# 87003697/DynamiCrafter

Measured on AMD Instinct MI355X. Metric: frames/sec (and denoising-step ms), 16f@576x1024, DDIM 50, higher is better.
Workload: dtype bf16; 1 GPU; inference_1024_v1.0.yaml: 1 clip/GPU, 16 frames, latent 72x128, DDIM 50 uniform_trailing eta=1, CFG 7.5 batched (cond+uncond), guidance_rescale 0.7, v-param+ZTSNR+dynamic rescale, hipGraph-captured step; clips_per_gpu=1, parallelism=dp1 over 1 distinct clips (no data-path collective), conditioning=local (1 rank), outputs_finite=True

## Files before the change

### dynamicrafter_amd/csrc/ff_fused.hip

```cpp
#include "attn_parts.h"
#include "dc_common.h"
#include "dcrafter_hip.h"
#include "lds_stage.h"
#include <stdint.h>
#include <type_traits>

namespace {

constexpr int FD = 320;
constexpr int FM = 4 * FD;
constexpr int FCH = 32;
constexpr int FNCH = FM / FCH;
constexpr int FBM = 128;
constexpr int W1_STAGE = 64 * FD * 2;
constexpr int W2_STAGE = FD * FCH * 2;
constexpr int W2_RING = 3;
constexpr int FF_LDS = 2 * W1_STAGE + W2_RING * W2_STAGE + 4 * 2048 + 2 * FM * 4;
static_assert(FF_LDS <= 160 * 1024, "LDS");

#ifdef DC_FF_STAMPS
__device__ unsigned long long g_ff_stamps[8];
#define FF_STAMP(i) do { asm volatile("s_waitcnt lgkmcnt(0)" ::: "memory"); const unsigned long long t__ = __builtin_readcyclecounter(); \
                         st_acc[i] += t__ - st_last; st_last = t__; } while (0)
#else
#define FF_STAMP(i) do { } while (0)
#endif

#ifdef DC_FF_GELU_ERF
#define FF_GELU(x) gelu_erf_f(x)
#else
#define FF_GELU(x) gelu_phi_f(x)
#endif

constexpr int LCH = 32;
constexpr int LW_STAGE = LCH * FD * 2;

template <int ROW_BYTES, int TILE_BYTES, bool PIN = true>
__device__ __forceinline__ void xs_piece_offsets(unsigned (&vo)[5], int wave, int lane) {
#pragma unroll
    for (int i = 0; i < 5; ++i) {
        const int u = wave * 5 + i;
        const int t = u >> 2, g = u & 3;
        vo[i] = (unsigned)((g * 8 + (lane >> 3)) * ROW_BYTES + t * TILE_BYTES + (((lane & 7) ^ ((g * 4 + (lane >> 4)) & 7)) << 4));
        if constexpr (PIN) asm volatile("" : "+v"(vo[i]));
    }
}
__device__ __forceinline__ unsigned xs_stage_dst(unsigned lds_base, int stage_off, int wave, int i) {
    return lds_base + stage_off + (wave * 5 + i) * 1024;
}
__device__ __forceinline__ void xs_issue_stage(unsigned lds_base, int stage_off, int wave, const unsigned (&vo)[5], uint64_t sbase) {
#pragma unroll
    for (int i = 0; i < 5; ++i) lds_dma16_sbase(xs_stage_dst(lds_base, stage_off, wave, i), vo[i], sbase);
}

template <int ROWS = 32>
__device__ __forceinline__ bf16x8_t xs_read_frag(const char* stage, int kk, int row, int fh) {
    return *(lds_vfrag_t*)((lds_char_t*)stage + (kk >> 2) * (ROWS * 128) + lds_off128(row, (kk & 3) * 2 + fh));
}

template <int PD, int NK, class Issue>
__device__ __forceinline__ void xs_stage_mma(const char* stage, const bf16x8_t (&xf)[NK], int k0, f32x16_t& acc, int fr, int fh,
                                             Issue&& issue) {
    bf16x8_t wr[PD];
#pragma unroll
    for (int kk = 0; kk < PD; ++kk) wr[kk] = xs_read_frag(stage, kk, fr, fh);
#pragma unroll
    for (int kk = 0; kk < FD / 16; ++kk) {
        bf16x8_t f = wr[kk % PD];
        if (kk + PD < FD / 16) wr[kk % PD] = xs_read_frag(stage, kk + PD, fr, fh);
        asm volatile("" : "+v"(f));
        acc = __builtin_amdgcn_mfma_f32_32x32x16_bf16(f, xf[k0 + kk], acc, 0, 0, 0);
        if (kk < 5) issue(kk);
    }
}

struct XsRowsLinear {
    int m0, M;
    __device__ __forceinline__ bool ok(int r) const { return m0 + r < M; }
    __device__ __forceinline__ size_t operator()(int r) const { return (size_t)(m0 + r); }
    __device__ __forceinline__ size_t clamped(int r) const { int m = m0 + r; if (m >= M) m = M - 1; return (size_t)m; }
};
struct XsRowsGather {
    int b, HW, p0;
    __device__ __forceinline__ bool ok(int) const { return true; }
    __device__ __forceinline__ size_t operator()(int r) const { return ((size_t)(b * 16 + (r & 15))) * HW + p0 + (r >> 4); }
    __device__ __forceinline__ size_t clamped(int r) const { return (*this)(r); }
};

template <int NK>
__device__ __forceinline__ void xs_load_rows(bf16x8_t (&xf)[NK], const bf16_t* xrow) {
#pragma unroll
    for (int kk = 0; kk < NK; ++kk) xf[kk] = *reinterpret_cast<const bf16x8_t*>(xrow + kk * 16);
}

__device__ __forceinline__ void xs_stage_ln_affine(float* lns, int KD, const float* g, const float* b, int tid) {
    for (int i = tid; i < KD; i += 256) { lns[i] = g[i]; lns[KD + i] = b[i]; }
}
__device__ __forceinline__ void xs_stage_gn_affine(float* lns, int KD, const float* g, const float* b, const float2* stats, int groups,
                                                   int tid) {
    for (int i = tid; i < KD; i += 256) {
        const float2 st = stats[i / (KD / groups)];
        const float a = g[i] * st.y;
        lns[i] = a; lns[KD + i] = b[i] - st.x * a;
    }
}
__device__ __forceinline__ void xs_stage_bias(float* bls, const float* bias, int N, int tid) {
    for (int i = tid; i < N; i += 256) bls[i] = bias[i];
}

__device__ __forceinline__ uint2* xs_patch_acc(char* ebuf, int fr, int fh, int q) {
    return reinterpret_cast<uint2*>(ebuf + fr * 64 + (((2 * q + fh) ^ (((fr >> 1) & 3) << 1)) << 3));
}
__device__ __forceinline__ u32x4_t* xs_patch_row(char* ebuf, int r, int rc) {
    return reinterpret_cast<u32x4_t*>(ebuf + r * 64 + ((rc ^ ((r >> 1) & 3)) << 4));
}
template <class Rows>
__device__ __forceinline__ void xs_load_chunk_rows(u32x4_t (&d)[2], const bf16_t* R, int ldr, const Rows& rows, int n0, int lane) {
#pragma unroll
    for (int t = 0; t < 2; ++t)
        d[t] = *reinterpret_cast<const u32x4_t*>(R + rows.clamped(t * 16 + (lane >> 2)) * ldr + n0 + (lane & 3) * 8);
}
__device__ __forceinline__ void xs_add_bf16x8(u32x4_t& d, const u32x4_t& rr) {
#pragma unroll
    for (int e = 0; e < 4; ++e) d[e] = add_bf2(d[e], rr[e]);
}
__device__ __forceinline__ void xs_add_bf16x4(float4& bv, uint2 rv) {
    bv.x += __uint_as_float(rv.x << 16); bv.y += __uint_as_float(rv.x & 0xffff0000u);
    bv.z += __uint_as_float(rv.y << 16); bv.w += __uint_as_float(rv.y & 0xffff0000u);
}
__device__ __forceinline__ uint2 xs_pack_acc(const f32x16_t& acc, int q, const float4& bv) {
    uint2 pk;
    pk.x = pack_bf2(acc[4 * q] + bv.x, acc[4 * q + 1] + bv.y);
    pk.y = pack_bf2(acc[4 * q + 2] + bv.z, acc[4 * q + 3] + bv.w);
    return pk;
}

struct XsPart { int tile, c_begin, c_end; };
__device__ __forceinline__ XsPart xs_part_decode(int nsplit, int cpp, int nch) {
    const int bgrp = (int)blockIdx.x / (8 * nsplit), brem = (int)blockIdx.x - bgrp * (8 * nsplit);
    const int part = brem >> 3;
    XsPart s;
    s.tile = bgrp * 8 + (brem & 7);
    s.c_begin = part * cpp;
    s.c_end = s.c_begin + cpp;
    if (s.c_end > nch) s.c_end = nch;
    return s;
}

template <int KD>
__device__ __forceinline__ void ln_rows_inplace(bf16x8_t (&xf)[KD / 16], const float* ln_g, const float* ln_b, float eps, int fh) {
    float sum = 0.f;
#pragma unroll
    for (int kk = 0; kk < KD / 16; ++kk) {
        const u32x4_t w = __builtin_bit_cast(u32x4_t, xf[kk]);
#pragma unroll
        for (int e = 0; e < 4; ++e) sum += __uint_as_float(w[e] << 16) + __uint_as_float(w[e] & 0xffff0000u);
    }
    sum += __shfl_xor(sum, 32, 64);
    const float mean = sum * (1.0f / KD);
#pragma unroll
    for (int kk = 0; kk < KD / 16; ++kk) asm volatile("" : "+v"(xf[kk]));
    float q = 0.f;
#pragma unroll
    for (int kk = 0; kk < KD / 16; ++kk) {
        const u32x4_t w = __builtin_bit_cast(u32x4_t, xf[kk]);
#pragma unroll
        for (int e = 0; e < 4; ++e) {
            const float d0 = __uint_as_float(w[e] << 16) - mean, d1 = __uint_as_float(w[e] & 0xffff0000u) - mean;
            q += d0 * d0 + d1 * d1;
        }
    }
    q += __shfl_xor(q, 32, 64);
    const float rstd = rsqrtf(q * (1.0f / KD) + eps);
#pragma unroll
    for (int kk = 0; kk < KD / 16; ++kk) asm volatile("" : "+v"(xf[kk]));
#pragma unroll
    for (int kk = 0; kk < KD / 16; ++kk) {
        if (kk % 5 == 0) asm volatile("" ::: "memory");
        const u32x4_t w = __builtin_bit_cast(u32x4_t, xf[kk]);
        const int c0 = kk * 16 + fh * 8;
        const float4 g0 = *reinterpret_cast<const float4*>(ln_g + c0), g1 = *reinterpret_cast<const float4*>(ln_g + c0 + 4);
        const float4 b0 = *reinterpret_cast<const float4*>(ln_b + c0), b1 = *reinterpret_cast<const float4*>(ln_b + c0 + 4);
        u32x4_t o;
        o[0] = pack_bf2((__uint_as_float(w[0] << 16) - mean) * rstd * g0.x + b0.x, (__uint_as_float(w[0] & 0xffff0000u) - mean) * rstd * g0.y + b0.y);
        o[1] = pack_bf2((__uint_as_float(w[1] << 16) - mean) * rstd * g0.z + b0.z, (__uint_as_float(w[1] & 0xffff0000u) - mean) * rstd * g0.w + b0.w);
        o[2] = pack_bf2((__uint_as_float(w[2] << 16) - mean) * rstd * g1.x + b1.x, (__uint_as_float(w[2] & 0xffff0000u) - mean) * rstd * g1.y + b1.y);
        o[3] = pack_bf2((__uint_as_float(w[3] << 16) - mean) * rstd * g1.z + b1.z, (__uint_as_float(w[3] & 0xffff0000u) - mean) * rstd * g1.w + b1.w);
        xf[kk] = __builtin_bit_cast(bf16x8_t, o);
        asm volatile("" : "+v"(xf[kk]));
    }
}

template <int KD, bool SILU = false>
__device__ __forceinline__ void affine_rows_inplace(bf16x8_t (&xf)[KD / 16], const float* a, const float* b, int fh) {
#pragma unroll
    for (int kk = 0; kk < KD / 16; ++kk) {
        if (kk % 5 == 0) asm volatile("" ::: "memory");
        const u32x4_t w = __builtin_bit_cast(u32x4_t, xf[kk]);
        const int c0 = kk * 16 + fh * 8;
        const float4 g0 = *reinterpret_cast<const float4*>(a + c0), g1 = *reinterpret_cast<const float4*>(a + c0 + 4);
        const float4 b0 = *reinterpret_cast<const float4*>(b + c0), b1 = *reinterpret_cast<const float4*>(b + c0 + 4);
        float v[8] = {__uint_as_float(w[0] << 16) * g0.x + b0.x, __uint_as_float(w[0] & 0xffff0000u) * g0.y + b0.y,
                      __uint_as_float(w[1] << 16) * g0.z + b0.z, __uint_as_float(w[1] & 0xffff0000u) * g0.w + b0.w,
                      __uint_as_float(w[2] << 16) * g1.x + b1.x, __uint_as_float(w[2] & 0xffff0000u) * g1.y + b1.y,
                      __uint_as_float(w[3] << 16) * g1.z + b1.z, __uint_as_float(w[3] & 0xffff0000u) * g1.w + b1.w};
        if constexpr (SILU) {
#pragma unroll
            for (int e = 0; e < 8; ++e) v[e] = silu_f(v[e]);
        }
        u32x4_t o;
#pragma unroll
        for (int e = 0; e < 4; ++e) o[e] = pack_bf2(v[2 * e], v[2 * e + 1]);
        xf[kk] = __builtin_bit_cast(bf16x8_t, o);
        asm volatile("" : "+v"(xf[kk]));
    }
}

struct FfParams {
    const bf16_t* X; int ldx;
    const bf16_t* W1;
    const float* b1;
    const bf16_t* W2p;
    const float* b2;
    const bf16_t* R; int ldr;
    bf16_t* O; int ldo;
    int M;
    const float* ln_g;
    const float* ln_b;
    float ln_eps;
    const bf16_t* Wp; const float* bp; const bf16_t* R2; int ldr2; bf16_t* O2; int ldo2;
};

template <bool LN, bool PROJ>
__global__ __launch_bounds__(256, 1) __attribute__((amdgpu_waves_per_eu(1, 1)))
void ff_geglu_fused320_kernel(const FfParams p) {
    extern __shared__ __attribute__((aligned(16))) char smem[];
    const int tid = threadIdx.x;
    const int lane = tid & 63;
    const int wave = __builtin_amdgcn_readfirstlane(tid >> 6);
    const int fr = lane & 31, fh = lane >> 5;
    const unsigned lds_base = (unsigned)(unsigned long)((lds_char_t*)smem);
    char* const w1s = smem;
    char* const w2s = smem + 2 * W1_STAGE;
    char* const ebuf = smem + 2 * W1_STAGE + W2_RING * W2_STAGE + wave * 2048;

    const int tiles = (p.M + FBM - 1) / FBM;
    float* const b1s = reinterpret_cast<float*>(smem + 2 * W1_STAGE + W2_RING * W2_STAGE + 4 * 2048);
    for (int i = tid; i < 2 * FM; i += 256) b1s[i] = p.b1[i];
    __syncthreads();

    unsigned vo1[10], vo2[5];
#pragma unroll
    for (int i = 0; i < 10; ++i) {
        const int u = wave * 10 + i;
        const int t = u >> 3, g = u & 7;
        const int row = (g < 4 ? g * 8 : FM + (g - 4) * 8) + (lane >> 3);
        vo1[i] = (unsigned)(row * (FD * 2) + t * 128 + (((lane & 7) ^ ((g * 4 + (lane >> 4)) & 7)) << 4));
    }
#pragma unroll
    for (int i = 0; i < 5; ++i)
        vo2[i] = (unsigned)(((wave * 5 + i) * 16 + (lane >> 2)) * (FM * 2) + (((lane & 3) ^ ((lane >> 4) & 3)) << 4));
#pragma unroll
    for (int i = 0; i < 10; ++i) asm volatile("" : "+v"(vo1[i]));
#pragma unroll
    for (int i = 0; i < 5; ++i) asm volatile("" : "+v"(vo2[i]));
    auto w1_base = [&](int j) { return (uint64_t)(uintptr_t)p.W1 + (uint64_t)j * (FCH * FD * 2); };
    auto w2_base = [&](int j) { return (uint64_t)(uintptr_t)p.W2p + (uint64_t)j * (FCH * 2); };
    auto w1_dst = [&](int j, int i) { return lds_base + (j & 1) * W1_STAGE + (wave * 10 + i) * 1024; };
    auto w2_dst = [&](int stage, int i) { return lds_base + 2 * W1_STAGE + stage * W2_STAGE + (wave * 5 + i) * 1024; };
    auto issue_w1 = [&](int j) __attribute__((always_inline)) {
#pragma unroll
        for (int i = 0; i < 10; ++i) lds_dma16_sbase(w1_dst(j, i), vo1[i], w1_base(j));
    };
    auto issue_w2 = [&](int j, int stage) __attribute__((always_inline)) {
#pragma unroll
        for (int i = 0; i < 5; ++i) lds_dma16_sbase(w2_dst(stage, i), vo2[i], w2_base(j));
    };

#ifdef DC_FF_STAMPS
    unsigned long long st_acc[5] = {0, 0, 0, 0, 0}, st_last = 0;
#endif
    for (int tile = blockIdx.x; tile < tiles; tile += gridDim.x) {
        const int m0 = tile * FBM + wave * 32;
        const XsRowsLinear rows{m0, p.M};
        bf16x8_t xf[FD / 16];
        xs_load_rows(xf, p.X + rows.clamped(fr) * p.ldx + fh * 8);
        if constexpr (LN) ln_rows_inplace<FD>(xf, p.ln_g, p.ln_b, p.ln_eps, fh);
        f32x16_t acc[FD / 32];
#pragma unroll
        for (int nb = 0; nb < FD / 32; ++nb)
#pragma unroll
            for (int r = 0; r < 16; ++r) acc[nb][r] = 0.f;

        constexpr int PD = 4, PD2 = 6;
        auto rd1 = [&](const char* s1, bf16x8_t (&wv)[PD], bf16x8_t (&wg)[PD], int kk, int slot) __attribute__((always_inline)) {
            wv[slot] = xs_read_frag<64>(s1, kk, fr, fh);
            wg[slot] = xs_read_frag<64>(s1, kk, 32 + fr, fh);
        };
        auto phase1 = [&](int c, f32x16_t& av, f32x16_t& ag) __attribute__((always_inline)) {
// ... 161 lines not shown
        wait_vmcnt<0>();
        __builtin_amdgcn_s_barrier();
        asm volatile("" ::: "memory");
        issue_w1(1);
        issue_w2(0, 0);
        f32x16_t a0, a0g, a1, a1g;
        bf16x8_t pf[2];
        phase1(0, a0, a0g);
        auto top = [&]() __attribute__((always_inline)) {
            FF_STAMP(4);
            wait_vmcnt<0>();
            __builtin_amdgcn_s_barrier();
            asm volatile("" ::: "memory");
            FF_STAMP(0);
        };
        top();
        issue_w1(2);
        issue_w2(1, 1);
        phase1_geglu(0, a0, a0g, a1, a1g, pf);
        FF_STAMP(2);
        int st = 0;
        auto body = [&](int j, const f32x16_t& cv, const f32x16_t& cg, f32x16_t& nv, f32x16_t& ng, auto DW1, auto DW2)
            __attribute__((always_inline)) {
            top();
            const int st2 = st + 2 >= W2_RING ? st + 2 - W2_RING : st + 2;
            phase2(st, pf, DW1, DW2, j, st2);
            st = st + 1 >= W2_RING ? 0 : st + 1;
            FF_STAMP(3);
            phase1_geglu(j, cv, cg, nv, ng, pf);
            FF_STAMP(2);
        };
        for (int j = 1; j < FNCH - 3; j += 2) {
            body(j, a1, a1g, a0, a0g, yes_t(), yes_t());
            body(j + 1, a0, a0g, a1, a1g, yes_t(), yes_t());
        }
        body(FNCH - 3, a1, a1g, a0, a0g, yes_t(), yes_t());
        body(FNCH - 2, a0, a0g, a1, a1g, no_t(), yes_t());
        top();
        phase2(st, pf, no_t(), no_t(), 0, 0);
        st = st + 1 >= W2_RING ? 0 : st + 1;
        geglu(FNCH - 1, a1, a1g, pf);
        phase2(st, pf, no_t(), no_t(), 0, 0);
        if constexpr (!PROJ) {
            int lane_e = lane;
            asm volatile("" : "+v"(lane_e));
            const int fr_e = lane_e & 31, fh_e = lane_e >> 5;
            const int rrow = lane_e >> 2, rc = lane_e & 3;
#pragma unroll
            for (int nb = 0; nb < FD / 32; ++nb) {
#pragma unroll
                for (int q = 0; q < 4; ++q) {
                    const float4 bv = *reinterpret_cast<const float4*>(p.b2 + nb * 32 + 8 * q + 4 * fh_e);
                    *xs_patch_acc(ebuf, fr_e, fh_e, q) = xs_pack_acc(acc[nb], q, bv);
                }
#pragma unroll
                for (int t = 0; t < 2; ++t) {
                    const int r = t * 16 + rrow;
                    u32x4_t d = *xs_patch_row(ebuf, r, rc);
                    if (!rows.ok(r)) continue;
                    const size_t m = rows(r);
                    const int n = nb * 32 + rc * 8;
                    if (p.R) xs_add_bf16x8(d, *reinterpret_cast<const u32x4_t*>(p.R + m * p.ldr + n));
                    *reinterpret_cast<u32x4_t*>(p.O + m * p.ldo + n) = d;
                }
            }
        } else {
            int lane_e = lane;
            asm volatile("" : "+v"(lane_e));
            const int fr_e = lane_e & 31, fh_e = lane_e >> 5;
            unsigned vo3[5];
            xs_piece_offsets<FD * 2, 128, false>(vo3, wave, lane_e);
            {
                const bf16_t* rrow = p.R + rows.clamped(fr_e) * p.ldr + 4 * fh_e;
#pragma unroll
                for (int nb = 0; nb < FD / 32; ++nb) {
                    u32x4_t fw[2];
#pragma unroll
                    for (int q = 0; q < 4; ++q) {
                        const int n = nb * 32 + 8 * q;
                        const float4 bv = *reinterpret_cast<const float4*>(p.b2 + n + 4 * fh_e);
                        const uint2 rr = *reinterpret_cast<const uint2*>(rrow + n);
                        const unsigned d0 = pack_bf2(acc[nb][4 * q] + bv.x, acc[nb][4 * q + 1] + bv.y);
                        const unsigned d1 = pack_bf2(acc[nb][4 * q + 2] + bv.z, acc[nb][4 * q + 3] + bv.w);
                        fw[q >> 1][2 * (q & 1)] = add_bf2(d0, rr.x);
                        fw[q >> 1][2 * (q & 1) + 1] = add_bf2(d1, rr.y);
                    }
                    xf[2 * nb] = __builtin_bit_cast(bf16x8_t, fw[0]);
                    xf[2 * nb + 1] = __builtin_bit_cast(bf16x8_t, fw[1]);
                }
            }
            wait_vmcnt<0>();
            __builtin_amdgcn_s_barrier();
            asm volatile("" ::: "memory");
            auto wp_base = [&](int c) { return (uint64_t)(uintptr_t)p.Wp + (uint64_t)c * (32 * FD * 2); };
            auto wp_off = [&](int c) { return 2 * W1_STAGE + (c & 1) * W2_STAGE; };
            xs_issue_stage(lds_base, wp_off(0), wave, vo3, wp_base(0));
            const bool full_tile = tile * FBM + FBM <= p.M;
            constexpr int PD3 = 6;
            for (int c = 0; c < FD / 32; ++c) {
                if (c == 0 || !full_tile) wait_vmcnt<0>();
                else wait_vmcnt<4>();
                __builtin_amdgcn_s_barrier();
                asm volatile("" ::: "memory");
                f32x16_t ya;
#pragma unroll
                for (int r = 0; r < 16; ++r) ya[r] = 0.f;
                const bool more = c + 1 < FD / 32;
                const uint64_t nbase = wp_base(c + 1);
                xs_stage_mma<PD3>(w2s + (c & 1) * W2_STAGE, xf, 0, ya, fr_e, fh_e, [&](int i) __attribute__((always_inline)) {
                    if (more) lds_dma16_sbase(xs_stage_dst(lds_base, wp_off(c + 1), wave, i), vo3[i], nbase);
                });
                const int n0 = c * 32;
#pragma unroll
                for (int q = 0; q < 4; ++q) {
                    const float4 bv = *reinterpret_cast<const float4*>(p.bp + n0 + 8 * q + 4 * fh_e);
                    *xs_patch_acc(ebuf, fr_e, fh_e, q) = xs_pack_acc(ya, q, bv);
                }
                const int rrow2 = lane_e >> 2, rc = lane_e & 3;
                u32x4_t rres[2];
                xs_load_chunk_rows(rres, p.R2, p.ldr2, rows, n0, lane_e);
#pragma unroll
                for (int t = 0; t < 2; ++t) {
                    const int r = t * 16 + rrow2;
                    u32x4_t d = *xs_patch_row(ebuf, r, rc);
                    xs_add_bf16x8(d, rres[t]);
                    if (rows.ok(r)) *reinterpret_cast<u32x4_t*>(p.O2 + rows(r) * p.ldo2 + n0 + rc * 8) = d;
                }
            }
            wait_vmcnt<0>();
        }
    }
#ifdef DC_FF_STAMPS
    if (blockIdx.x == 0 && tid == 0)
        for (int i = 0; i < 5; ++i) atomicAdd(&g_ff_stamps[i], st_acc[i]);
#endif
}


constexpr int LL_BIAS = 640;
constexpr int ll_lds(int kh) { return 2 * LW_STAGE + 4 * 2048 + 2 * FD * kh * 4 + LL_BIAS * 4; }

struct LlParams {
    const bf16_t* X; int ldx;
    const bf16_t* W;
    const float* bias;
    bf16_t* O; int ldo;
    int M, N;
    int nsplit, cpp;
    const float* ln_g; const float* ln_b; float ln_eps;
    const float2* gn_stats; int gn_groups, gn_rpi;
    const bf16_t* R; int ldr;
};

template <int NORM, int KH, bool RES = false>
__global__ __launch_bounds__(256, KH == 1 ? 3 : 2)
void norm_linear_kernel(const LlParams p) {
    constexpr int KD = FD * KH;
    extern __shared__ __attribute__((aligned(16))) char smem[];
    const int tid = threadIdx.x;
    const int lane = tid & 63;
    const int wave = __builtin_amdgcn_readfirstlane(tid >> 6);
    const int fr = lane & 31, fh = lane >> 5;
    const unsigned lds_base = (unsigned)(unsigned long)((lds_char_t*)smem);
    char* const ebuf = smem + 2 * LW_STAGE + wave * 2048;
    const XsPart part = xs_part_decode(p.nsplit, p.cpp, p.N / LCH);
    const int tile = part.tile, c_begin = part.c_begin, c_end = part.c_end;
    if (tile * FBM >= p.M) return;
    const XsRowsLinear rows{tile * FBM + wave * 32, p.M};
    const bool full_tile = tile * FBM + FBM <= p.M;
    if (c_begin >= c_end) return;

    unsigned vo[5];
    xs_piece_offsets<KD * 2, 128>(vo, wave, lane);
    auto w_base = [&](int c, int h) { return (uint64_t)(uintptr_t)p.W + (uint64_t)c * (LCH * KD * 2) + h * (FD * 2); };
    xs_issue_stage(lds_base, 0, wave, vo, w_base(c_begin, 0));

    bf16x8_t xf[KD / 16];
    float* const lns = reinterpret_cast<float*>(smem + 2 * LW_STAGE + 4 * 2048);
    float* const bls = lns + 2 * KD;
    const bool bias_lds = p.bias != nullptr && p.N <= LL_BIAS;
    xs_load_rows(xf, p.X + rows.clamped(fr) * p.ldx + fh * 8);
    if (bias_lds) xs_stage_bias(bls, p.bias, p.N, tid);
    if constexpr (NORM == 1) xs_stage_ln_affine(lns, KD, p.ln_g, p.ln_b, tid);
    if constexpr (NORM == 2) {
        const int inst = (int)(((long long)tile * FBM) / p.gn_rpi);
        xs_stage_gn_affine(lns, KD, p.ln_g, p.ln_b, p.gn_stats + (size_t)inst * p.gn_groups, p.gn_groups, tid);
    }
    asm volatile("s_waitcnt vmcnt(0) lgkmcnt(0)" ::: "memory");
    __builtin_amdgcn_s_barrier();
    asm volatile("" ::: "memory");
    if constexpr (NORM == 1) ln_rows_inplace<KD>(xf, lns, lns + KD, p.ln_eps, fh);
    if constexpr (NORM == 2) affine_rows_inplace<KD>(xf, lns, lns + KD, fh);

    constexpr int PD = 6;
    int slot = 0;
    for (int c = c_begin; c < c_end; ++c) {
        f32x16_t acc;
#pragma unroll
        for (int r = 0; r < 16; ++r) acc[r] = 0.f;
        u32x4_t rres[2];
#pragma unroll
        for (int h = 0; h < KH; ++h) {
            if (c > c_begin || h > 0) {
                if (!full_tile) wait_vmcnt<0>();
                else if (h == 0) wait_vmcnt<2>();
                else wait_vmcnt<0>();
                __builtin_amdgcn_s_barrier();
                asm volatile("" ::: "memory");
            }
            if constexpr (RES) {
                if (h == 0) xs_load_chunk_rows(rres, p.R, p.ldr, rows, c * LCH, lane);
            }
            const bool more = h + 1 < KH || c + 1 < c_end;
            const uint64_t nb = h + 1 < KH ? w_base(c, h + 1) : w_base(c + 1, 0);
            xs_stage_mma<PD>(smem + slot * LW_STAGE, xf, h * (FD / 16), acc, fr, fh, [&](int i) __attribute__((always_inline)) {
                if (more) lds_dma16_sbase(xs_stage_dst(lds_base, (slot ^ 1) * LW_STAGE, wave, i), vo[i], nb);
            });
            slot ^= 1;
        }
        {
            const int n0 = c * LCH;
            const int rrow = lane >> 2, rc = lane & 3;
            if constexpr (RES) {
#pragma unroll
                for (int t = 0; t < 2; ++t) *xs_patch_row(ebuf, t * 16 + rrow, rc) = rres[t];
            }
#pragma unroll
            for (int q = 0; q < 4; ++q) {
                float4 bv = {0.f, 0.f, 0.f, 0.f};
                if (bias_lds) bv = *reinterpret_cast<const float4*>(bls + n0 + 8 * q + 4 * fh);
                else if (p.bias) bv = *reinterpret_cast<const float4*>(p.bias + n0 + 8 * q + 4 * fh);
                uint2* const slot = xs_patch_acc(ebuf, fr, fh, q);
                if constexpr (RES) xs_add_bf16x4(bv, *slot);
                *slot = xs_pack_acc(acc, q, bv);
            }
#pragma unroll
            for (int t = 0; t < 2; ++t) {
                const int r = t * 16 + rrow;
                const u32x4_t d = *xs_patch_row(ebuf, r, rc);
                if (rows.ok(r)) *reinterpret_cast<u32x4_t*>(p.O + rows(r) * p.ldo + n0 + rc * 8) = d;
            }
        }
    }
}


constexpr int TA_PATCH = 32 * ATTN_VLD;
constexpr int ta_ring(int kh) { return kh == 1 ? 2 : 4; }
constexpr int ta_lds(int kh) { return ta_ring(kh) * LW_STAGE + 4 * TA_PATCH + 2 * FD * kh * 4; }

struct TaParams {
    const bf16_t* X; int ldx;
    const bf16_t* W;
    bf16_t* O; int ldo;
    const float* ln_g; const float* ln_b; float ln_eps;
    int HW;
    float c;
};

template <int KH>
__global__ __launch_bounds__(256, KH == 1 ? 2 : 1)
void ln_qkv_tattn_kernel(const TaParams p) {
    constexpr int KD = FD * KH;
    constexpr int NS = ta_ring(KH);
    constexpr int SPH = 6 * KH;
    static_assert(SPH % NS == 0, "ring phase");
    extern __shared__ __attribute__((aligned(16))) char smem[];
    const int tid = threadIdx.x;
    const int lane = tid & 63;
    const int wave = __builtin_amdgcn_readfirstlane(tid >> 6);
    const int fr = lane & 31, fh = lane >> 5;
    const unsigned lds_base = (unsigned)(unsigned long)((lds_char_t*)smem);
    char* const vpatch = smem + NS * LW_STAGE + wave * TA_PATCH;
    float* const lns = reinterpret_cast<float*>(smem + NS * LW_STAGE + 4 * TA_PATCH);
    const int gpb = p.HW >> 3;
    const int b = (int)blockIdx.x / gpb, p0 = ((int)blockIdx.x - b * gpb) * 8 + 2 * wave;
    const XsRowsGather grow{b, p.HW, p0};

    unsigned vo[5];
    xs_piece_offsets<KD * 2, 128>(vo, wave, lane);
    auto w_base = [&](int h, int part, int kh) {
        return (uint64_t)(uintptr_t)p.W + (uint64_t)((part >> 1) * KD + 64 * h + 32 * (part & 1)) * (KD * 2) + (uint64_t)kh * (FD * 2);
    };

    const int hpw = 5 * KH / (int)gridDim.y;
    const int h_begin = (int)blockIdx.y * hpw, h_end = h_begin + hpw;
#pragma unroll
    for (int d = 0; d < NS - 1; ++d) xs_issue_stage(lds_base, d * LW_STAGE, wave, vo, w_base(h_begin + d / SPH, (d % SPH) / KH, d % KH));

    bf16x8_t xf[KD / 16];
    xs_load_rows(xf, p.X + grow(fr) * p.ldx + fh * 8);
    xs_stage_ln_affine(lns, KD, p.ln_g, p.ln_b, tid);
    asm volatile("s_waitcnt vmcnt(0) lgkmcnt(0)" ::: "memory");
    __builtin_amdgcn_s_barrier();
    asm volatile("" ::: "memory");
    ln_rows_inplace<KD>(xf, lns, lns + KD, p.ln_eps, fh);

    constexpr int PD = 6;
    const int tr_off = attn_vt_lane_off(lane);
    const int px = fr >> 4;
    for (int h = h_begin; h < h_end; ++h) {
        bf16x8_t qf[4], kf[4];
#pragma unroll
        for (int part = 0; part < 6; ++part) {
            f32x16_t acc;
#pragma unroll
            for (int r = 0; r < 16; ++r) acc[r] = 0.f;
#pragma unroll
            for (int kh = 0; kh < KH; ++kh) {
                const int lin = part * KH + kh;
                const int slot = lin % NS;
                if (h > h_begin || lin > 0) {
                    const int rem = (h + 1 == h_end) ? SPH - 1 - lin : NS;
                    const int younger = rem < NS - 2 ? rem : NS - 2;
                    const int n = 5 * younger + ((lin == 0) ? 4 : 0);
                    if (n >= 14) wait_vmcnt<14>();
                    else if (n >= 10) wait_vmcnt<10>();
                    else if (n >= 5) wait_vmcnt<5>();
                    else if (n >= 4) wait_vmcnt<4>();
                    else wait_vmcnt<0>();
                    __builtin_amdgcn_s_barrier();
                    asm volatile("" ::: "memory");
                }
                const int nl = lin + NS - 1;
                const int nh = h + nl / SPH;
                const bool more = nh < h_end;
                const uint64_t nb = w_base(nh, (nl % SPH) / KH, nl % KH);
                xs_stage_mma<PD>(smem + slot * LW_STAGE, xf, kh * (FD / 16), acc, fr, fh, [&](int i) __attribute__((always_inline)) {
                    if (more) lds_dma16_sbase(xs_stage_dst(lds_base, (nl % NS) * LW_STAGE, wave, i), vo[i], nb);
                });
            }
            if (part < 4) {
#pragma unroll
                for (int s2 = 0; s2 < 2; ++s2) {
                    if (part < 2) qf[2 * (part & 1) + s2] = attn_pack_p(acc, s2);
                    else kf[2 * (part & 1) + s2] = attn_pack_p(acc, s2);
                }
            } else {
#pragma unroll
                for (int q = 0; q < 4; ++q) {
                    uint2 pk;
                    pk.x = pack_bf2(acc[4 * q], acc[4 * q + 1]);
                    pk.y = pack_bf2(acc[4 * q + 2], acc[4 * q + 3]);
                    *reinterpret_cast<uint2*>(vpatch + fr * ATTN_VLD + (32 * (part & 1) + 8 * q + 4 * fh) * 2) = pk;
                }
            }
        }
        f32x16_t sc;
#pragma unroll
        for (int r = 0; r < 16; ++r) sc[r] = 0.f;
#pragma unroll
        for (int j = 0; j < 4; ++j) sc = __builtin_amdgcn_mfma_f32_32x32x16_bf16(kf[j], qf[j], sc, 0, 0, 0);
        float mx = -1e30f;
#pragma unroll
        for (int r = 0; r < 16; ++r) {
            if ((r >> 3) != px) sc[r] = -1e30f;
            mx = fmaxf(mx, sc[r]);
        }
        mx = fmaxf(mx, __shfl_xor(mx, 32, 64));
        float sum = 0.f;
#pragma unroll
        for (int r = 0; r < 16; ++r) {
            sc[r] = __builtin_amdgcn_exp2f((sc[r] - mx) * p.c);
            sum += sc[r];
        }
        sum += __shfl_xor(sum, 32, 64);
        const float inv = 1.0f / sum;
        bf16x8_t pf[2];
#pragma unroll
        for (int ks = 0; ks < 2; ++ks) {
            u32x4_t pw;
#pragma unroll
            for (int e = 0; e < 4; ++e) pw[e] = pack_bf2(sc[8 * ks + 2 * e] * inv, sc[8 * ks + 2 * e + 1] * inv);
            pf[ks] = __builtin_bit_cast(bf16x8_t, pw);
        }
        __builtin_amdgcn_s_waitcnt(0xc07f);
        __builtin_amdgcn_wave_barrier();
        f32x16_t oacc[2];
#pragma unroll
        for (int db = 0; db < 2; ++db) {
#pragma unroll
            for (int r = 0; r < 16; ++r) oacc[db][r] = 0.f;
#pragma unroll
            for (int ks = 0; ks < 2; ++ks) {
                const bf16x8_t vf = attn_vt_frag((const lds_char_t*)(vpatch + (16 * ks + 4 * fh) * ATTN_VLD + db * 64 + tr_off));
                oacc[db] = __builtin_amdgcn_mfma_f32_32x32x16_bf16(vf, pf[ks], oacc[db], 0, 0, 0);
            }
        }
#pragma unroll
        for (int db = 0; db < 2; ++db)
#pragma unroll
            for (int q = 0; q < 4; ++q) {
                uint2 pk;
                pk.x = pack_bf2(oacc[db][4 * q], oacc[db][4 * q + 1]);
// ... 43 lines not shown
    const int tile = part.tile, c_begin = part.c_begin, c_end = part.c_end;
    if (tile >= p.ntiles) return;
    const int gpb = p.HW >> 3;
    const int b = tile / gpb, p0 = (tile - b * gpb) * 8 + 2 * wave;
    const XsRowsGather grow{b, p.HW, p0};
    if (c_begin >= c_end) return;

    unsigned vo[5];
    xs_piece_offsets<3 * KD * 2, 384>(vo, wave, lane);
    auto w_base = [&](int c, int j) {
        const int jt = j / KH, h = j - jt * KH;
        const int tap = jt == 0 ? 1 : (jt == 1 ? 0 : 2);
        return (uint64_t)(uintptr_t)p.W + (uint64_t)c * (LCH * 3 * KD * 2) + tap * 128 + h * (5 * 384);
    };
    xs_issue_stage(lds_base, 0, wave, vo, w_base(c_begin, 0));

    bf16x8_t xf[KD / 16];
    xs_load_rows(xf, p.X + grow(fr) * p.ldx + fh * 8);
    xs_stage_gn_affine(lns, KD, p.gn_g, p.gn_b, p.gn_stats + (size_t)b * p.gn_groups, p.gn_groups, tid);
    if (bias_lds) xs_stage_bias(bls, p.bias, p.N, tid);
    asm volatile("s_waitcnt vmcnt(0) lgkmcnt(0)" ::: "memory");
    __builtin_amdgcn_s_barrier();
    asm volatile("" ::: "memory");
    affine_rows_inplace<KD, true>(xf, lns, lns + KD, fh);

    constexpr int PD = KH == 1 ? 6 : 3;
    constexpr int NS = 3 * KH;
    int slot = 0;
    for (int c = c_begin; c < c_end; ++c) {
        f32x16_t out, y;
        u32x4_t rres[2];
#pragma unroll
        for (int j = 0; j < NS; ++j) {
            const int jt = j / KH, h = j % KH;
            if (c > c_begin || j > 0) {
                if (j == 0) { if (RES && KH != 1) wait_vmcnt<4>(); else wait_vmcnt<2>(); }
                else wait_vmcnt<0>();
                __builtin_amdgcn_s_barrier();
                asm volatile("" ::: "memory");
            }
            if constexpr (RES && KH == 1) {
                if (j == 0) {
#pragma unroll
                    for (int t = 0; t < 2; ++t)
                        rres[t] = *reinterpret_cast<const u32x4_t*>(p.R + grow(t * 16 + (lane >> 2)) * p.ldr + c * LCH + (lane & 3) * 8);
                }
            }
            f32x16_t& acc = jt == 0 ? out : y;
            if (h == 0) {
#pragma unroll
                for (int r = 0; r < 16; ++r) acc[r] = 0.f;
            }
            const bool more = j + 1 < NS || c + 1 < c_end;
            const uint64_t nb = j + 1 < NS ? w_base(c, j + 1) : w_base(c + 1, 0);
            xs_stage_mma<PD>(smem + slot * LW_STAGE, xf, h * (FD / 16), acc, fr, fh, [&](int i) __attribute__((always_inline)) {
                if (more) lds_dma16_sbase(xs_stage_dst(lds_base, (slot ^ 1) * LW_STAGE, wave, i), vo[i], nb);
            });
            slot ^= 1;
            if (jt > 0 && h == KH - 1) {
#pragma unroll
                for (int r = 0; r < 16; ++r) {
                    const float yv = y[r];
                    out[r] += __int_as_float(jt == 1 ? __builtin_amdgcn_update_dpp(0, __float_as_int(yv), 0x111, 0xf, 0xf, false)
                                                     : __builtin_amdgcn_update_dpp(0, __float_as_int(yv), 0x101, 0xf, 0xf, false));
                }
            }
        }
        {
            const int n0 = c * LCH;
            const int rrow = lane >> 2, rc = lane & 3;
            if constexpr (RES) {
                if constexpr (KH != 1) {
#pragma unroll
                    for (int t = 0; t < 2; ++t) rres[t] = *reinterpret_cast<const u32x4_t*>(p.R + grow(t * 16 + rrow) * p.ldr + n0 + rc * 8);
                }
#pragma unroll
                for (int t = 0; t < 2; ++t) *xs_patch_row(ebuf, t * 16 + rrow, rc) = rres[t];
            }
#pragma unroll
            for (int q = 0; q < 4; ++q) {
                float4 bv = bias_lds ? *reinterpret_cast<const float4*>(bls + n0 + 8 * q + 4 * fh)
                                     : *reinterpret_cast<const float4*>(p.bias + n0 + 8 * q + 4 * fh);
                uint2* const slot2 = xs_patch_acc(ebuf, fr, fh, q);
                if constexpr (RES) xs_add_bf16x4(bv, *slot2);
                *slot2 = xs_pack_acc(out, q, bv);
            }
#pragma unroll
            for (int t = 0; t < 2; ++t) {
                const int r = t * 16 + rrow;
                const u32x4_t d = *xs_patch_row(ebuf, r, rc);
                *reinterpret_cast<u32x4_t*>(p.O + grow(r) * p.ldo + n0 + rc * 8) = d;
            }
        }
    }
}

}

#ifdef DC_FF_STAMPS
extern "C" int dc_ff_debug_stamps(unsigned long long* out, int reset) {
    hipError_t e = hipMemcpyFromSymbol(out, HIP_SYMBOL(g_ff_stamps), sizeof(unsigned long long) * 8);
    if (e == hipSuccess && reset) {
        unsigned long long z[8] = {0};
        e = hipMemcpyToSymbol(HIP_SYMBOL(g_ff_stamps), z, sizeof(z));
    }
    return (int)e;
}
#endif

template <bool LN, bool PROJ>
static int launch_ff_fused(const FfParams& p, hipStream_t stream) {
    static DcLdsOnce lds_once;
    if (const int e = lds_once.ensure(reinterpret_cast<const void*>(&ff_geglu_fused320_kernel<LN, PROJ>), FF_LDS)) return e;
    const int tiles = (p.M + FBM - 1) / FBM;
    hipLaunchKernelGGL((ff_geglu_fused320_kernel<LN, PROJ>), dim3(tiles < 256 ? tiles : 256), dim3(256), FF_LDS, stream, p);
    DC_CHECK_LAUNCH();
    return 0;
}

static int ff_fused_common(const uint16_t* x, int ldx, const float* ln_gamma, const float* ln_beta, float ln_eps,
                           const uint16_t* w1, const float* b1, const uint16_t* w2p, const float* b2, const uint16_t* residual,
                           int ldr, uint16_t* out, int ldo, const uint16_t* wp, const float* bp, const uint16_t* residual2,
                           int ldr2, uint16_t* out2, int ldo2, int M, hipStream_t stream) {
    FfParams p;
    p.X = x; p.ldx = ldx; p.W1 = w1; p.b1 = b1; p.W2p = w2p; p.b2 = b2; p.R = residual; p.ldr = ldr; p.O = out; p.ldo = ldo;
    p.M = M; p.ln_g = ln_gamma; p.ln_b = ln_beta; p.ln_eps = ln_eps;
    p.Wp = wp; p.bp = bp; p.R2 = residual2; p.ldr2 = ldr2; p.O2 = out2; p.ldo2 = ldo2;
    if (wp) return ln_gamma ? launch_ff_fused<true, true>(p, stream) : launch_ff_fused<false, true>(p, stream);
    return ln_gamma ? launch_ff_fused<true, false>(p, stream) : launch_ff_fused<false, false>(p, stream);
}

extern "C" int dc_ff_geglu_fused320(const uint16_t* x, int ldx, const float* ln_gamma, const float* ln_beta, float ln_eps,
                                    const uint16_t* w1, const float* b1, const uint16_t* w2p, const float* b2,
                                    const uint16_t* residual, int ldr, uint16_t* out, int ldo, int M, void* stream_) {
    if (!x || !w1 || !b1 || !w2p || !b2 || !out || ((ln_gamma == nullptr) != (ln_beta == nullptr))) return DC_ERR_ARG;
    if (M < 1 || ldx % 8 || ldo % 8 || (residual && ldr % 8)) return DC_ERR_SHAPE;
    if (((uintptr_t)x | (uintptr_t)out | (uintptr_t)w1 | (uintptr_t)w2p | (uintptr_t)(residual ? residual : out)) % 16) return DC_ERR_SHAPE;
    return ff_fused_common(x, ldx, ln_gamma, ln_beta, ln_eps, w1, b1, w2p, b2, residual, ldr, out, ldo, nullptr, nullptr,
                           nullptr, 0, nullptr, 0, M, (hipStream_t)stream_);
}

extern "C" int dc_ff_geglu_proj_fused320(const uint16_t* x, int ldx, const float* ln_gamma, const float* ln_beta, float ln_eps,
                                         const uint16_t* w1, const float* b1, const uint16_t* w2p, const float* b2,
                                         const uint16_t* wp, const float* bp, const uint16_t* residual2, int ldr2,
                                         uint16_t* out, int ldo, int M, void* stream_) {
    if (!x || !w1 || !b1 || !w2p || !b2 || !wp || !bp || !residual2 || !out || ((ln_gamma == nullptr) != (ln_beta == nullptr)))
        return DC_ERR_ARG;
    if (M < 1 || ldx % 8 || ldo % 8 || ldr2 % 8) return DC_ERR_SHAPE;
    if (((uintptr_t)x | (uintptr_t)out | (uintptr_t)w1 | (uintptr_t)w2p | (uintptr_t)wp | (uintptr_t)residual2) % 16) return DC_ERR_SHAPE;
    return ff_fused_common(x, ldx, ln_gamma, ln_beta, ln_eps, w1, b1, w2p, b2, x, ldx, nullptr, 0, wp, bp, residual2, ldr2, out,
                           ldo, M, (hipStream_t)stream_);
}

template <int NORM, int KH, bool RES = false>
static int launch_norm_linear_t(const LlParams& p, dim3 grid, hipStream_t stream) {
    static DcLdsOnce lds_once;
    if (const int e = lds_once.ensure(reinterpret_cast<const void*>(&norm_linear_kernel<NORM, KH, RES>), ll_lds(KH))) return e;
    hipLaunchKernelGGL((norm_linear_kernel<NORM, KH, RES>), grid, dim3(256), ll_lds(KH), stream, p);
    DC_CHECK_LAUNCH();
    return 0;
}

struct XsSplit { int nsplit, cpp; dim3 grid; };
static XsSplit xs_split_n(int tiles, int nch, int slots) {
    int nsplit = 1;
    while (tiles * nsplit < 3 * slots && nsplit * 2 <= nch && nch / (nsplit * 2) >= 5) nsplit *= 2;
    return {nsplit, (nch + nsplit - 1) / nsplit, dim3((unsigned)((tiles + 7) / 8 * 8 * nsplit))};
}

static int launch_norm_linear(int norm, int K, LlParams& p, hipStream_t stream) {
    const XsSplit sp = xs_split_n((p.M + FBM - 1) / FBM, p.N / LCH, 256 * (K == FD ? 3 : 2));
    p.nsplit = sp.nsplit;
    p.cpp = sp.cpp;
    const dim3 grid = sp.grid;
    if (p.R) return K == FD ? launch_norm_linear_t<0, 1, true>(p, grid, stream) : launch_norm_linear_t<0, 2, true>(p, grid, stream);
    if (K == FD) {
        if (norm == 1) return launch_norm_linear_t<1, 1>(p, grid, stream);
        if (norm == 2) return launch_norm_linear_t<2, 1>(p, grid, stream);
        return launch_norm_linear_t<0, 1>(p, grid, stream);
    }
    if (norm == 1) return launch_norm_linear_t<1, 2>(p, grid, stream);
    if (norm == 2) return launch_norm_linear_t<2, 2>(p, grid, stream);
    return launch_norm_linear_t<0, 2>(p, grid, stream);
}

static int ll_params(LlParams& p, const uint16_t* x, int ldx, int K, const uint16_t* w, const float* bias, uint16_t* out, int ldo,
                     int M, int N) {
    if ((K != FD && K != 2 * FD) || M < 1 || N < LCH || N % LCH || ldx % 8 || ldo % 8) return DC_ERR_SHAPE;
    if (((uintptr_t)x | (uintptr_t)out | (uintptr_t)w) % 16) return DC_ERR_SHAPE;
    p.X = x; p.ldx = ldx; p.W = w; p.bias = bias; p.O = out; p.ldo = ldo; p.M = M; p.N = N;
    p.ln_g = nullptr; p.ln_b = nullptr; p.ln_eps = 0.f; p.gn_stats = nullptr; p.gn_groups = 1; p.gn_rpi = FBM;
    p.R = nullptr; p.ldr = 0;
    return 0;
}

extern "C" int dc_ln_linear(const uint16_t* x, int ldx, int K, const float* ln_gamma, const float* ln_beta, float ln_eps,
                            const uint16_t* w, const float* bias, uint16_t* out, int ldo, int M, int N, void* stream_) {
    if (!x || !w || !out || ((ln_gamma == nullptr) != (ln_beta == nullptr))) return DC_ERR_ARG;
    LlParams p;
    if (const int e = ll_params(p, x, ldx, K, w, bias, out, ldo, M, N)) return e;
    p.ln_g = ln_gamma; p.ln_b = ln_beta; p.ln_eps = ln_eps;
    return launch_norm_linear(ln_gamma ? 1 : 0, K, p, (hipStream_t)stream_);
}

extern "C" int dc_linear_residual(const uint16_t* x, int ldx, int K, const uint16_t* w, const float* bias,
                                  const uint16_t* residual, int ldr, uint16_t* out, int ldo, int M, int N, void* stream_) {
    if (!x || !w || !out || !residual) return DC_ERR_ARG;
    LlParams p;
    if (const int e = ll_params(p, x, ldx, K, w, bias, out, ldo, M, N)) return e;
    if (ldr % 8 || (uintptr_t)residual % 16) return DC_ERR_SHAPE;
    p.R = residual; p.ldr = ldr;
    return launch_norm_linear(0, K, p, (hipStream_t)stream_);
}

extern "C" int dc_gn_linear(const uint16_t* x, int ldx, int K, const float* gamma, const float* beta, const float* stats,
                            int groups, int rows_per_inst, const uint16_t* w, const float* bias, uint16_t* out, int ldo,
                            int M, int N, void* stream_) {
    if (!x || !w || !out || !gamma || !beta || !stats) return DC_ERR_ARG;
    LlParams p;
    if (const int e = ll_params(p, x, ldx, K, w, bias, out, ldo, M, N)) return e;
    if (groups < 1 || K % groups || rows_per_inst < FBM || rows_per_inst % FBM || M % rows_per_inst) return DC_ERR_SHAPE;
    p.ln_g = gamma; p.ln_b = beta;
    p.gn_stats = reinterpret_cast<const float2*>(stats); p.gn_groups = groups; p.gn_rpi = rows_per_inst;
    return launch_norm_linear(2, K, p, (hipStream_t)stream_);
}

template <int KH>
static int launch_ln_qkv_tattn(const uint16_t* x, int ldx, const float* ln_gamma, const float* ln_beta, float ln_eps,
                               const uint16_t* wqkv, uint16_t* out, int ldo, int B, int T, int HW, float scale, void* stream_) {
    if (!x || !ln_gamma || !ln_beta || !wqkv || !out) return DC_ERR_ARG;
    if (B < 1 || T != 16 || HW < 8 || HW % 8 || ldx % 8 || ldo % 8) return DC_ERR_SHAPE;
    if (((uintptr_t)x | (uintptr_t)out | (uintptr_t)wqkv) % 16) return DC_ERR_SHAPE;
    static DcLdsOnce lds_once;
    if (const int e = lds_once.ensure(reinterpret_cast<const void*>(&ln_qkv_tattn_kernel<KH>), ta_lds(KH))) return e;
    TaParams p;
    p.X = x; p.ldx = ldx; p.W = wqkv; p.O = out; p.ldo = ldo; p.ln_g = ln_gamma; p.ln_b = ln_beta; p.ln_eps = ln_eps;
    p.HW = HW; p.c = scale * 1.4426950408889634f;
    static const int hsplit_env = [] { const char* e = getenv("DC_TA_HSPLIT"); return e ? atoi(e) : 0; }();
    const int hsplit = (KH == 2 && hsplit_env == 2) ? 2 : 1;
    hipLaunchKernelGGL(ln_qkv_tattn_kernel<KH>, dim3((unsigned)(B * (HW / 8)), hsplit), dim3(256), ta_lds(KH), (hipStream_t)stream_, p);
    DC_CHECK_LAUNCH();
    return 0;
}

extern "C" int dc_ln_qkv_temporal_attn320(const uint16_t* x, int ldx, const float* ln_gamma, const float* ln_beta, float ln_eps,
                                          const uint16_t* wqkv, uint16_t* out, int ldo, int B, int T, int HW, float scale,
                                          void* stream_) {
    return launch_ln_qkv_tattn<1>(x, ldx, ln_gamma, ln_beta, ln_eps, wqkv, out, ldo, B, T, HW, scale, stream_);
}

extern "C" int dc_ln_qkv_temporal_attn640(const uint16_t* x, int ldx, const float* ln_gamma, const float* ln_beta, float ln_eps,
                                          const uint16_t* wqkv, uint16_t* out, int ldo, int B, int T, int HW, float scale,
                                          void* stream_) {
    return launch_ln_qkv_tattn<2>(x, ldx, ln_gamma, ln_beta, ln_eps, wqkv, out, ldo, B, T, HW, scale, stream_);
}

template <int KH, bool RES>
static int launch_gn_silu_tconv(const TcParams& p, dim3 grid, hipStream_t stream) {
    static DcLdsOnce lds_once;
    if (const int e = lds_once.ensure(reinterpret_cast<const void*>(&gn_silu_tconv_kernel<KH, RES>), ll_lds(KH))) return e;
    hipLaunchKernelGGL((gn_silu_tconv_kernel<KH, RES>), grid, dim3(256), ll_lds(KH), stream, p);
    DC_CHECK_LAUNCH();
    return 0;
}

extern "C" int dc_gn_silu_tconv3(const uint16_t* x, int ldx, int C, const float* gamma, const float* beta, const float* stats,
                                 int groups, const uint16_t* w, const float* bias, const uint16_t* residual, int ldr,
                                 uint16_t* out, int ldo, int B, int T, int HW, int N, void* stream_) {
    if (!x || !gamma || !beta || !stats || !w || !bias || !out) return DC_ERR_ARG;
    if ((C != FD && C != 2 * FD) || B < 1 || T != 16 || HW < 8 || HW % 8 || N < LCH || N % LCH || ldx % 8 || ldo % 8 ||
        (residual && ldr % 8)) return DC_ERR_SHAPE;
    if (groups < 1 || C % groups) return DC_ERR_SHAPE;
    if (((uintptr_t)x | (uintptr_t)out | (uintptr_t)w | (uintptr_t)(residual ? residual : out)) % 16) return DC_ERR_SHAPE;
    TcParams p;
    p.X = x; p.ldx = ldx; p.W = w; p.bias = bias; p.R = residual; p.ldr = ldr; p.O = out; p.ldo = ldo;
    p.gn_g = gamma; p.gn_b = beta; p.gn_stats = reinterpret_cast<const float2*>(stats); p.gn_groups = groups; p.HW = HW; p.N = N;
    p.ntiles = B * (HW / 8);
    const XsSplit sp = xs_split_n(p.ntiles, N / LCH, 256 * 2);
    p.nsplit = sp.nsplit; p.cpp = sp.cpp;
    const dim3 grid = sp.grid;
    hipStream_t stream = (hipStream_t)stream_;
    if (C == FD) return residual ? launch_gn_silu_tconv<1, true>(p, grid, stream) : launch_gn_silu_tconv<1, false>(p, grid, stream);
    return residual ? launch_gn_silu_tconv<2, true>(p, grid, stream) : launch_gn_silu_tconv<2, false>(p, grid, stream);
}
```

Measured before the change: 2.643 frames/s.

## Make norm_linear kernel persistent with next-tile X prefetch and double-buffered registers

Converts the norm+linear GEMM kernel into a persistent grid-stride loop sized to CU count. Each block walks several row tiles and prefetches the next tile's X rows and weight stage while finishing the current one, optionally into a second register set (XB) for K=320. This is meant to hide per-block startup latency (X loads, LN/GN affine staging, first weight stage) and cut block launch overhead. Large-N biased calls are split into chunks so the bias always fits in LDS. The cost is lower occupancy for XB variants (launch bounds drop from 3 to 2), more register pressure, and extra GN-affine restaging logic.

```diff
diff --git a/dynamicrafter_amd/csrc/ff_fused.hip b/dynamicrafter_amd/csrc/ff_fused.hip
--- a/dynamicrafter_amd/csrc/ff_fused.hip
+++ b/dynamicrafter_amd/csrc/ff_fused.hip
@@ -136,8 +136,8 @@
 }
 
 struct XsPart { int tile, c_begin, c_end; };
-__device__ __forceinline__ XsPart xs_part_decode(int nsplit, int cpp, int nch) {
-    const int bgrp = (int)blockIdx.x / (8 * nsplit), brem = (int)blockIdx.x - bgrp * (8 * nsplit);
+__device__ __forceinline__ XsPart xs_part_decode(int bid, int nsplit, int cpp, int nch) {
+    const int bgrp = bid / (8 * nsplit), brem = bid - bgrp * (8 * nsplit);
     const int part = brem >> 3;
     XsPart s;
     s.tile = bgrp * 8 + (brem & 7);
@@ -145,6 +145,9 @@
     s.c_end = s.c_begin + cpp;
     if (s.c_end > nch) s.c_end = nch;
     return s;
+}
+__device__ __forceinline__ XsPart xs_part_decode(int nsplit, int cpp, int nch) {
+    return xs_part_decode((int)blockIdx.x, nsplit, cpp, nch);
 }
 
 template <int KD>
@@ -612,9 +615,10 @@
     const bf16_t* R; int ldr;
 };
 
-template <int NORM, int KH, bool RES = false>
-__global__ __launch_bounds__(256, KH == 1 ? 3 : 2)
+template <int NORM, int KH, bool RES = false, bool XB = false>
+__global__ __launch_bounds__(256, (KH == 1 && !XB) ? 3 : 2)
 void norm_linear_kernel(const LlParams p) {
+    static_assert(!XB || KH == 1, "a second X register set at K = 640 is 320 registers");
     constexpr int KD = FD * KH;
     extern __shared__ __attribute__((aligned(16))) char smem[];
     const int tid = threadIdx.x;
@@ -623,11 +627,12 @@
     const int fr = lane & 31, fh = lane >> 5;
     const unsigned lds_base = (unsigned)(unsigned long)((lds_char_t*)smem);
     char* const ebuf = smem + 2 * LW_STAGE + wave * 2048;
-    const XsPart part = xs_part_decode(p.nsplit, p.cpp, p.N / LCH);
-    const int tile = part.tile, c_begin = part.c_begin, c_end = part.c_end;
+    int bid = (int)blockIdx.x;
+    const XsPart part = xs_part_decode(bid, p.nsplit, p.cpp, p.N / LCH);
+    const int c_begin = part.c_begin, c_end = part.c_end;
+    int tile = part.tile;
     if (tile * FBM >= p.M) return;
-    const XsRowsLinear rows{tile * FBM + wave * 32, p.M};
-    const bool full_tile = tile * FBM + FBM <= p.M;
+    XsRowsLinear rows{tile * FBM + wave * 32, p.M};
     if (c_begin >= c_end) return;
 
     unsigned vo[5];
@@ -638,68 +643,112 @@
     bf16x8_t xf[KD / 16];
     float* const lns = reinterpret_cast<float*>(smem + 2 * LW_STAGE + 4 * 2048);
     float* const bls = lns + 2 * KD;
-    const bool bias_lds = p.bias != nullptr && p.N <= LL_BIAS;
+    const bool has_bias = p.bias != nullptr;
     xs_load_rows(xf, p.X + rows.clamped(fr) * p.ldx + fh * 8);
-    if (bias_lds) xs_stage_bias(bls, p.bias, p.N, tid);
+    if (has_bias) xs_stage_bias(bls, p.bias, p.N, tid);
     if constexpr (NORM == 1) xs_stage_ln_affine(lns, KD, p.ln_g, p.ln_b, tid);
+    int inst = 0;
     if constexpr (NORM == 2) {
-        const int inst = (int)(((long long)tile * FBM) / p.gn_rpi);
+        inst = (int)(((long long)tile * FBM) / p.gn_rpi);
         xs_stage_gn_affine(lns, KD, p.ln_g, p.ln_b, p.gn_stats + (size_t)inst * p.gn_groups, p.gn_groups, tid);
     }
     asm volatile("s_waitcnt vmcnt(0) lgkmcnt(0)" ::: "memory");
     __builtin_amdgcn_s_barrier();
     asm volatile("" ::: "memory");
-    if constexpr (NORM == 1) ln_rows_inplace<KD>(xf, lns, lns + KD, p.ln_eps, fh);
-    if constexpr (NORM == 2) affine_rows_inplace<KD>(xf, lns, lns + KD, fh);
 
     constexpr int PD = 6;
     int slot = 0;
-    for (int c = c_begin; c < c_end; ++c) {
-        f32x16_t acc;
-#pragma unroll
-        for (int r = 0; r < 16; ++r) acc[r] = 0.f;
-        u32x4_t rres[2];
-#pragma unroll
-        for (int h = 0; h < KH; ++h) {
-            if (c > c_begin || h > 0) {
-                if (!full_tile) wait_vmcnt<0>();
-                else if (h == 0) wait_vmcnt<2>();
-                else wait_vmcnt<0>();
-                __builtin_amdgcn_s_barrier();
-                asm volatile("" ::: "memory");
-            }
-            if constexpr (RES) {
-                if (h == 0) xs_load_chunk_rows(rres, p.R, p.ldr, rows, c * LCH, lane);
-            }
-            const bool more = h + 1 < KH || c + 1 < c_end;
-            const uint64_t nb = h + 1 < KH ? w_base(c, h + 1) : w_base(c + 1, 0);
-            xs_stage_mma<PD>(smem + slot * LW_STAGE, xf, h * (FD / 16), acc, fr, fh, [&](int i) __attribute__((always_inline)) {
-                if (more) lds_dma16_sbase(xs_stage_dst(lds_base, (slot ^ 1) * LW_STAGE, wave, i), vo[i], nb);
-            });
-            slot ^= 1;
-        }
-        {
-            const int n0 = c * LCH;
-            const int rrow = lane >> 2, rc = lane & 3;
-            if constexpr (RES) {
-#pragma unroll
-                for (int t = 0; t < 2; ++t) *xs_patch_row(ebuf, t * 16 + rrow, rc) = rres[t];
-            }
-#pragma unroll
-            for (int q = 0; q < 4; ++q) {
-                float4 bv = {0.f, 0.f, 0.f, 0.f};
-                if (bias_lds) bv = *reinterpret_cast<const float4*>(bls + n0 + 8 * q + 4 * fh);
-                else if (p.bias) bv = *reinterpret_cast<const float4*>(p.bias + n0 + 8 * q + 4 * fh);
-                uint2* const slot = xs_patch_acc(ebuf, fr, fh, q);
-                if constexpr (RES) xs_add_bf16x4(bv, *slot);
-                *slot = xs_pack_acc(acc, q, bv);
-            }
-#pragma unroll
-            for (int t = 0; t < 2; ++t) {
-                const int r = t * 16 + rrow;
-                const u32x4_t d = *xs_patch_row(ebuf, r, rc);
-                if (rows.ok(r)) *reinterpret_cast<u32x4_t*>(p.O + rows(r) * p.ldo + n0 + rc * 8) = d;
-            }
+    for (;;) {
+        const bool full_tile = tile * FBM + FBM <= p.M;
+        if constexpr (NORM == 1) ln_rows_inplace<KD>(xf, lns, lns + KD, p.ln_eps, fh);
+        if constexpr (NORM == 2) affine_rows_inplace<KD>(xf, lns, lns + KD, fh);
+        bid += (int)gridDim.x;
+        const int tile_n = xs_part_decode(bid, p.nsplit, p.cpp, p.N / LCH).tile;
+        const bool has_next = (long long)tile_n * FBM < p.M;
+        const XsRowsLinear rows_n{has_next ? tile_n * FBM + wave * 32 : 0, p.M};
+        auto xrow_n = [&]() __attribute__((always_inline)) {
+            int m0n = rows_n.m0;
+            asm volatile("" : "+s"(m0n));
+            return p.X + XsRowsLinear{m0n, p.M}.clamped(fr) * p.ldx + fh * 8;
+        };
+        bf16x8_t xn[XB ? KD / 16 : 1];
+        if constexpr (XB) {
+            if (has_next) xs_load_rows(xn, xrow_n());
+        }
+        for (int c = c_begin; c < c_end; ++c) {
+            f32x16_t acc;
+#pragma unroll
+            for (int r = 0; r < 16; ++r) acc[r] = 0.f;
+            u32x4_t rres[2];
+            int m0c = rows.m0;
+            asm volatile("" : "+s"(m0c));
+            const XsRowsLinear crows{m0c, p.M};
+#pragma unroll
+            for (int h = 0; h < KH; ++h) {
+                if (c > c_begin || h > 0) {
+                    if (!full_tile) wait_vmcnt<0>();
+                    else if (h == 0) wait_vmcnt<2>();
+                    else wait_vmcnt<0>();
+                    __builtin_amdgcn_s_barrier();
+                    asm volatile("" ::: "memory");
+                }
+                if constexpr (RES) {
+                    if (h == 0) xs_load_chunk_rows(rres, p.R, p.ldr, crows, c * LCH, lane);
+                }
+                const bool more = h + 1 < KH || c + 1 < c_end || has_next;
+                const uint64_t nb = h + 1 < KH ? w_base(c, h + 1) : w_base(c + 1 < c_end ? c + 1 : c_begin, 0);
+                xs_stage_mma<PD>(smem + slot * LW_STAGE, xf, h * (FD / 16), acc, fr, fh, [&](int i) __attribute__((always_inline)) {
+                    if (more) lds_dma16_sbase(xs_stage_dst(lds_base, (slot ^ 1) * LW_STAGE, wave, i), vo[i], nb);
+                });
+                slot ^= 1;
+            }
+            {
+                const int n0 = c * LCH;
+                const int rrow = lane >> 2, rc = lane & 3;
+                if constexpr (RES) {
+#pragma unroll
+                    for (int t = 0; t < 2; ++t) *xs_patch_row(ebuf, t * 16 + rrow, rc) = rres[t];
+                }
+                if constexpr (!XB) {
+                    if (c + 1 == c_end && has_next) {
+                        asm volatile("" ::: "memory");
+                        xs_load_rows(xf, xrow_n());
+                    }
+                }
+#pragma unroll
+                for (int q = 0; q < 4; ++q) {
+                    float4 bv = {0.f, 0.f, 0.f, 0.f};
+                    if (has_bias) bv = *reinterpret_cast<const float4*>(bls + n0 + 8 * q + 4 * fh);
+                    uint2* const slot = xs_patch_acc(ebuf, fr, fh, q);
+                    if constexpr (RES) xs_add_bf16x4(bv, *slot);
+                    *slot = xs_pack_acc(acc, q, bv);
+                }
+#pragma unroll
+                for (int t = 0; t < 2; ++t) {
+                    const int r = t * 16 + rrow;
+                    const u32x4_t d = *xs_patch_row(ebuf, r, rc);
+                    if (crows.ok(r)) *reinterpret_cast<u32x4_t*>(p.O + crows(r) * p.ldo + n0 + rc * 8) = d;
+                }
+            }
+        }
+        if (!has_next) break;
+        tile = tile_n;
+        rows = rows_n;
+        if constexpr (NORM == 2) {
+            const int inst_n = (int)(((long long)tile * FBM) / p.gn_rpi);
+            if (inst_n != inst) {
+                inst = inst_n;
+                if ((c_end - c_begin) * KH < 2) __builtin_amdgcn_s_barrier();
+                xs_stage_gn_affine(lns, KD, p.ln_g, p.ln_b, p.gn_stats + (size_t)inst * p.gn_groups, p.gn_groups, tid);
+            }
+        }
+        if (full_tile) wait_vmcnt<2>(); else wait_vmcnt<0>();
+        if constexpr (NORM == 2) asm volatile("s_waitcnt lgkmcnt(0)" ::: "memory");
+        __builtin_amdgcn_s_barrier();
+        asm volatile("" ::: "memory");
+        if constexpr (XB) {
+#pragma unroll
+            for (int kk = 0; kk < KD / 16; ++kk) xf[kk] = xn[kk];
         }
     }
 }
@@ -1049,11 +1098,11 @@
                            ldo, M, (hipStream_t)stream_);
 }
 
-template <int NORM, int KH, bool RES = false>
+template <int NORM, int KH, bool RES = false, bool XB = false>
 static int launch_norm_linear_t(const LlParams& p, dim3 grid, hipStream_t stream) {
     static DcLdsOnce lds_once;
-    if (const int e = lds_once.ensure(reinterpret_cast<const void*>(&norm_linear_kernel<NORM, KH, RES>), ll_lds(KH))) return e;
-    hipLaunchKernelGGL((norm_linear_kernel<NORM, KH, RES>), grid, dim3(256), ll_lds(KH), stream, p);
+    if (const int e = lds_once.ensure(reinterpret_cast<const void*>(&norm_linear_kernel<NORM, KH, RES, XB>), ll_lds(KH))) return e;
+    hipLaunchKernelGGL((norm_linear_kernel<NORM, KH, RES, XB>), grid, dim3(256), ll_lds(KH), stream, p);
     DC_CHECK_LAUNCH();
     return 0;
 }
@@ -1065,11 +1114,45 @@
     return {nsplit, (nch + nsplit - 1) / nsplit, dim3((unsigned)((tiles + 7) / 8 * 8 * nsplit))};
 }
 
+static int xs_persist_mode() {
+    static const int v = [] { const char* e = getenv("DC_XS_PERSIST"); return e ? atoi(e) : 2; }();
+    return v;
+}
+static dim3 xs_persist_grid(const XsSplit& sp, int per_cu) {
+    static const int cus = [] {
+        int dev = 0, n = 0;
+        if (hipGetDevice(&dev) != hipSuccess || hipDeviceGetAttribute(&n, hipDeviceAttributeMultiprocessorCount, dev) != hipSuccess) n = 0;
+        return n > 0 ? n : 256;
+    }();
+    const unsigned g = 8u * (unsigned)sp.nsplit;
+    unsigned n = (unsigned)(cus * per_cu) / g * g;
+    if (n < g) n = g;
+    return dim3(n < sp.grid.x ? n : sp.grid.x);
+}
+
 static int launch_norm_linear(int norm, int K, LlParams& p, hipStream_t stream) {
     const XsSplit sp = xs_split_n((p.M + FBM - 1) / FBM, p.N / LCH, 256 * (K == FD ? 3 : 2));
     p.nsplit = sp.nsplit;
     p.cpp = sp.cpp;
-    const dim3 grid = sp.grid;
+    if (p.bias && p.N > LL_BIAS) {
+        for (int n0 = 0; n0 < p.N; n0 += LL_BIAS) {
+            LlParams q = p;
+            q.W += (size_t)n0 * K; q.bias += n0; q.O += n0; q.N = p.N - n0 < LL_BIAS ? p.N - n0 : LL_BIAS;
+            if (q.R) q.R += n0;
+            if (const int e = launch_norm_linear(norm, K, q, stream)) return e;
+        }
+        return 0;
+    }
+    const int mode = xs_persist_mode();
+    const bool xb = mode == 2 && K == FD;
+    const bool walk = mode == 1 || (mode == 2 && (K == FD || norm == 2));
+    const dim3 grid = walk ? xs_persist_grid(sp, K == FD && !xb ? 3 : 2) : sp.grid;
+    if (xb) {
+        if (p.R) return launch_norm_linear_t<0, 1, true, true>(p, grid, stream);
+        if (norm == 1) return launch_norm_linear_t<1, 1, false, true>(p, grid, stream);
+        if (norm == 2) return launch_norm_linear_t<2, 1, false, true>(p, grid, stream);
+        return launch_norm_linear_t<0, 1, false, true>(p, grid, stream);
+    }
     if (p.R) return K == FD ? launch_norm_linear_t<0, 1, true>(p, grid, stream) : launch_norm_linear_t<0, 2, true>(p, grid, stream);
     if (K == FD) {
         if (norm == 1) return launch_norm_linear_t<1, 1>(p, grid, stream);
```

Result: no change. 2.660 frames/s (median of 6 runs) (+0.6%).
